# Schatten2021/rust-raytracing

Hardware: AMD Instinct MI355X
Metric: Mrays/s (primary rays, whole node), 10k-sphere 1080p 64spp (higher is better)
Workload: dtype f64; 1 GPU; C2: 10k random spheres (scene seed 1), 1920x1080, 64 spp; width=1920, height=1080, rays_per_pixel=64, n_objects=10000, partition=single GPU

## Files before the change

rust-raytracing_amd/build.py:

```python
import hashlib
import os
import shutil
import subprocess
from concurrent.futures import ThreadPoolExecutor

HERE = os.path.dirname(os.path.abspath(__file__))
CSRC = os.path.join(HERE, "csrc")
LIB = os.path.join(HERE, "librtx_hip.so")
LAB_LIB = os.path.join(HERE, "librtx_hip_lab.so")
OBJ_DIR = os.path.join(HERE, "build")
SOURCES = ["rtx_kernels.hip", "rtx_bvh_spheres.hip", "rtx_bvh_mesh.hip", "rtx_wavefront.hip", "rtx_query.hip", "rtx_update.hip", "rtx_pack.hip",
           "rtx_api.hip", "rtx_api_update.hip", "rtx_api_debug.hip"]
HEADERS = ["rtx_math.h", "rtx_scene.h", "rtx_bvh.h", "rtx_device.h", "rtx_traverse.h", "rtx_mesh_step.h", "rtx_wavefront.h",
           "rtx_launch.h", "rtx_refit.h", "rtx_pack.h", "rtx_host.h"]
FLAGS = ["--offload-arch=gfx950", "-O3", "-std=c++17", "-fPIC", "-ffp-contract=off",
         "-fno-fast-math", "-Wall", "-Wno-unused-function"]
LAB_FLAGS = ["-DRTX_LAB"]


def hipcc():
    exe = shutil.which("hipcc") or "/opt/rocm/bin/hipcc"
    if not os.path.exists(exe):
        raise RuntimeError("hipcc not found: librtx_hip.so cannot be built (there is no CPU fallback)")
    return exe


def _input_files():
    files = [os.path.join(CSRC, f) for f in HEADERS]
    files.append(os.path.join(HERE, "..", "include", "rtx_hip.h"))
    return files


def _digest(source, flags):
    h = hashlib.sha256()
    h.update(" ".join(flags).encode())
    for f in [os.path.join(CSRC, source)] + _input_files():
        with open(f, "rb") as fh:
            h.update(fh.read())
    return h.hexdigest()[:20]


def build(force=False, extra_flags=(), verbose=False, lib=None, jobs=None, lab=False):
    if lib is None:
        lib = LAB_LIB if lab else LIB
    flags = FLAGS + (LAB_FLAGS if lab else []) + list(extra_flags)
    os.makedirs(OBJ_DIR, exist_ok=True)
    exe = hipcc()
    objs, todo = [], []
    for s in SOURCES:
        obj = os.path.join(OBJ_DIR, "%s.%s.o" % (s[:-4], _digest(s, flags)))
        objs.append(obj)
        if force or not os.path.exists(obj):
            todo.append((s, obj))

    def compile_one(job):
        s, obj = job
        cmd = [exe] + flags + ["-c", os.path.join(CSRC, s), "-o", obj + ".tmp"]
        if verbose:
            print(" ".join(cmd), flush=True)
        subprocess.check_call(cmd)
        os.replace(obj + ".tmp", obj)

    if todo:
        with ThreadPoolExecutor(max_workers=jobs or min(len(todo), max(1, (os.cpu_count() or 2) - 1))) as ex:
            list(ex.map(compile_one, todo))
    stamp = lib + ".objs"
    want = "\n".join(os.path.basename(o) for o in objs) + "\n"
    have = open(stamp).read() if os.path.exists(stamp) else None
    if todo or not os.path.exists(lib) or have != want:
        if os.path.exists(stamp):
            os.remove(stamp)
        cmd = [exe, "--offload-arch=gfx950", "-shared", "-fPIC", "-Wl,-Bsymbolic"] + objs + ["-o", lib + ".tmp"]
        if verbose:
            print(" ".join(cmd), flush=True)
        subprocess.check_call(cmd)
        os.replace(lib + ".tmp", lib)
        with open(stamp, "w") as fh:
            fh.write(want)
    if not extra_flags:
        keep = set()
        for st in os.listdir(HERE):
            if st.endswith(".so.objs") and os.path.exists(os.path.join(HERE, st[:-5])):
                keep.update(open(os.path.join(HERE, st)).read().split())
        for f in os.listdir(OBJ_DIR):
            if f.endswith(".o") and f not in keep:
                os.remove(os.path.join(OBJ_DIR, f))
    return lib


def build_all(force=False, verbose=False):
    return build(force=force, verbose=verbose), build(force=force, verbose=verbose, lab=True)


if __name__ == "__main__":
    import sys
    for path in build_all(force="--force" in sys.argv, verbose=True):
        print(path)
# ... 1 lines not shown
```

rust-raytracing_amd/csrc/rtx_bvh_spheres.hip:

```cpp
#include "rtx_launch.h"
#include "rtx_traverse.h"

#include <cmath>

namespace rtx {

#ifndef RTX_SPH_WAVES
#define RTX_SPH_WAVES 4
#endif
constexpr int kSphWavesPerSimd = RTX_SPH_WAVES;
constexpr int kSphStack = 30;

struct SphSurvivor {
    double px, py, pz, dx, dy, dz;
    uint32_t ridx;
    uint32_t first_id;
    uint64_t key;
};
static_assert(sizeof(SphSurvivor) == 64, "SphSurvivor must be one 64-byte line");
struct SphQueue {
    SphSurvivor *rec;
    const uint32_t *perm;
    unsigned long long *count;
    unsigned long long capacity;
    uint32_t cut_walkers;
};
constexpr uint32_t kSphQueueChunk = 512;
#ifndef RTX_SPH_CUT
#define RTX_SPH_CUT 24
#endif
#ifndef RTX_SPH_CUT_DONE
#define RTX_SPH_CUT_DONE 32
#endif
#ifndef RTX_SPH_LEAF_LANES
#define RTX_SPH_LEAF_LANES 8
#endif
#ifndef RTX_ROUND_GLOBAL
#define RTX_ROUND_GLOBAL 1
#endif
#ifndef RTX_ROUND_CARRY_KEY
#define RTX_ROUND_CARRY_KEY 1
#endif
#ifndef RTX_ROUND_DRAW
#define RTX_ROUND_DRAW 1
#endif
constexpr bool kRoundGlobal = RTX_ROUND_GLOBAL != 0;
constexpr uint32_t kSphLeafLanes = RTX_SPH_LEAF_LANES;
constexpr uint32_t kSphCutWalkers = RTX_SPH_CUT;
constexpr uint32_t kSphCutDone = RTX_SPH_CUT_DONE;

__device__ __forceinline__ void sph_queue_append(const SphQueue &sq, Counters *__restrict__ ctr, bool go, const RayState &r,
                                                 uint32_t ridx, uint32_t first_id, uint32_t lane,
                                                 unsigned long long &out_next, unsigned long long &out_end)
{
    const unsigned long long m = __ballot(go);
    const uint32_t n = (uint32_t)__popcll(m);
    if (n == 0u) return;
    const unsigned long long rem = out_end - out_next;
    unsigned long long base2 = 0;
    if (rem < (unsigned long long)n) {
        if (lane == 0) base2 = atomicAdd(sq.count, (unsigned long long)kSphQueueChunk);
        base2 = ((unsigned long long)__builtin_amdgcn_readfirstlane((uint32_t)(base2 >> 32)) << 32) |
                __builtin_amdgcn_readfirstlane((uint32_t)base2);
    }
    if (go) {
        const unsigned long long k = bvh_mbcnt(m);
        const unsigned long long slot = k < rem ? out_next + k : base2 + (k - rem);
        if (slot < sq.capacity) {
            double4 *p = reinterpret_cast<double4 *>(sq.rec + slot);
            p[0] = make_double4(r.pos.x, r.pos.y, r.pos.z, r.dir.x);
            uint2 tail;
            tail.x = ridx; tail.y = first_id;
#if RTX_ROUND_CARRY_KEY
            p[1] = make_double4(r.dir.y, r.dir.z, __longlong_as_double(((long long)tail.y << 32) | (long long)tail.x),
                                __longlong_as_double((long long)r.key));
#else
            p[1] = make_double4(r.dir.y, r.dir.z, __longlong_as_double(((long long)tail.y << 32) | (long long)tail.x), 0.0);
#endif
        } else {
            atomicAdd(&ctr[1].pad_, 1ull);
        }
    }
    if (rem < (unsigned long long)n) { out_next = base2 + ((unsigned long long)n - rem); out_end = base2 + kSphQueueChunk; }
// ... 176 lines not shown
            }
            if (RTX_SPH_PROFILE == 8 && alive && !midwalk && walked && !overflow) rtx_prof += qcnt;
        }
#endif
        if (alive && !midwalk) {
            Hit h;
            hit_init(h);
            ++segs;
            box_tests += nbox;
            leaf_filters += nleaf;
            if (walked && !overflow) {
#pragma unroll 1
                for (uint32_t e = 0; e < qcnt; ++e) {
                    if (__uint_as_float(lq[(size_t)(kSphQueue + e) * kBvhThreads + tid]) <= best_up) {
                        const uint32_t idx = lq[(size_t)e * kBvhThreads + tid];
                        double t;
                        if (sphere_distance(la.spheres[idx], rx, &t)) hit_consider(h, t, la.sphere_ids[idx], 0, idx);
                        exact += 1;
                    }
                }
            } else {
                for (uint32_t k = 0; k < sv.n_spheres; ++k) {
                    double t;
                    if (sphere_distance(la.spheres[k], rx, &t)) hit_consider(h, t, la.sphere_ids[k], 0, k);
                }
                exact += sv.n_spheres;
            }
            for (uint32_t k = 0; k < sv.n_planes; ++k) {
                double t;
                if (plane_distance(sv.planes[k], rx, &t)) hit_consider(h, t, sv.planes[k].id, 1, k);
            }
            for (uint32_t k = 0; k < sv.n_tri_filter; ++k) {
                const uint32_t tk = la.tri_fidx[k];
                double t;
                if (triangle_distance(la.tris[tk], rx, &t)) hit_consider(h, t, la.tris[tk].id, 2, tk);
            }
            exact += sv.n_planes + sv.n_tri_filter;

            bool done = true;
            if (h.id != kNone) {
#if RTX_ROUND_DRAW
                r.draw = 6u + 2u * r.bounce;
#endif
                advance_and_shade<kRoundGlobal>(sv, h, r);
                first_id = h.id;
                done = (r.bounce >= bounce_limit) || light_is_zero(r);
            }
            if (done) {
                store_sample<kRoundGlobal>(samples, rv, ridx, r.result);
                alive = false;
            }
        }
        if constexpr (MODE == 1) {
            sph_queue_append(sq, ctr, alive, r, ridx, first_id, lane, out_next, out_end);
            alive = false;
        }
    }
    if constexpr (MODE == 1) sph_queue_close(sq, lane, out_next, out_end);
#if defined(RTX_LAB) && defined(RTX_SPH_PROFILE)
    if (MODE == 2) exact = rtx_prof;
#endif
    unsigned long long filt = box_tests + leaf_filters;
#pragma unroll
    for (int off = 32; off > 0; off >>= 1) {
        segs += __shfl_xor(segs, off, 64);
        exact += __shfl_xor(exact, off, 64);
        filt += __shfl_xor(filt, off, 64);
        box_tests += __shfl_xor(box_tests, off, 64);
    }
    if (lane == 0) {
        const uint32_t shard = (blockIdx.x * (kBvhThreads >> 6) + (tid >> 6)) & (kCounterShards - 1);
        if (segs) atomicAdd(&ctr[shard].segments, segs);
        if (exact) atomicAdd(&ctr[shard].exact_tests, exact);
        if (filt) atomicAdd(&ctr[shard].filter_tests, filt);
        if (box_tests) atomicAdd(&ctr[2 + (shard % (kCounterShards - 2))].pad_, box_tests);
    }
}

constexpr int kSpkStack = 63;
#ifndef RTX_SPK_WAVES
#define RTX_SPK_WAVES 4
#endif
constexpr int kSpkWaves = RTX_SPK_WAVES;
#ifdef RTX_LAB
constexpr uint32_t kSphNoPackets = 1u;
#endif



template <int SGN>
__device__ __forceinline__ void sph_packet_walk(const PkConst4 cnodes, const PkConst4 csph, const PkConstU32 cprims, uint32_t root,
                                                const Ray32S &q, const SphereRay &sr, uint32_t *lq, uint32_t tid, uint32_t lane,
                                                float &best_up, uint32_t &qcnt, bool &overflow, uint32_t &nbox, uint32_t &nleaf)
{
    int stk = 0;
    uint32_t sp = 0, node = __builtin_amdgcn_readfirstlane(root);
    while (node != kNone) {
        const PkConst4 np = cnodes + 8 * (size_t)node;
        float4 a[4], b[4];
#pragma unroll
        for (int c = 0; c < 4; ++c) { a[c] = np[c]; b[c] = np[4 + c]; }
        uint32_t lnk[4], cnt[4];
        float tc[4];
        unsigned long long hm[4];
#pragma unroll
        for (int c = 0; c < 4; ++c) {
            lnk[c] = pk_bits(a[c].w);
            cnt[c] = pk_bits(b[c].w);
            float tn, tf;
            if (SGN < 8) {
                const float nx_ = (SGN & 1) ? b[c].x : a[c].x, fx_ = (SGN & 1) ? a[c].x : b[c].x;
                const float ny_ = (SGN & 2) ? b[c].y : a[c].y, fy_ = (SGN & 2) ? a[c].y : b[c].y;
                const float nz_ = (SGN & 4) ? b[c].z : a[c].z, fz_ = (SGN & 4) ? a[c].z : b[c].z;
                tn = fmaxf(fmaxf(__builtin_fmaf(nx_, q.ix, q.nx), __builtin_fmaf(ny_, q.iy, q.ny)), fmaxf(__builtin_fmaf(nz_, q.iz, q.nz), 0.0f));
                tf = fminf(fminf(__builtin_fmaf(fx_, q.ix, q.nx), __builtin_fmaf(fy_, q.iy, q.ny)), __builtin_fmaf(fz_, q.iz, q.nz));
            } else {
                const float x0 = __builtin_fmaf(a[c].x, q.ix, q.nx), x1 = __builtin_fmaf(b[c].x, q.ix, q.nx);
                const float y0 = __builtin_fmaf(a[c].y, q.iy, q.ny), y1 = __builtin_fmaf(b[c].y, q.iy, q.ny);
                const float z0 = __builtin_fmaf(a[c].z, q.iz, q.nz), z1 = __builtin_fmaf(b[c].z, q.iz, q.nz);
                tn = fmaxf(fmaxf(fminf(x0, x1), fminf(y0, y1)), fmaxf(fminf(z0, z1), 0.0f));
                tf = fminf(fminf(fmaxf(x0, x1), fmaxf(y0, y1)), fmaxf(z0, z1));
            }
            tc[c] = __builtin_fmaf(tn, 1.0f - 4.76837158e-7f, -q.e);
            const float tf_hi = __builtin_fmaf(tf, 1.0f + 4.76837158e-7f, q.e);
            hm[c] = __builtin_amdgcn_ballot_w64(tc[c] <= fminf(tf_hi, best_up));
        }
        if (best_up >= 0.0f) nbox += 4;
        if (((cnt[0] | cnt[1] | cnt[2] | cnt[3]) & 0xFFFFu) != 0u) {
            uint32_t leafmask = 0;
#pragma unroll
            for (int c = 0; c < 4; ++c)
                if (cnt[c] - 1u < 0xFFFFu && hm[c] != 0ull) leafmask |= 1u << c;
            while (leafmask != 0u) {
                const uint32_t c = (uint32_t)__builtin_ctz(leafmask);
                leafmask &= leafmask - 1u;
                const uint32_t first = c == 0 ? lnk[0] : (c == 1 ? lnk[1] : (c == 2 ? lnk[2] : lnk[3]));
                const uint32_t n = (c == 0 ? cnt[0] : (c == 1 ? cnt[1] : (c == 2 ? cnt[2] : cnt[3]))) & 0xFFFFu;
                const unsigned long long m = c == 0 ? hm[0] : (c == 1 ? hm[1] : (c == 2 ? hm[2] : hm[3]));
                const bool in = ((m >> lane) & 1ull) != 0ull;
                if (in) nleaf += n;
                for (uint32_t j = 0; j < n; ++j) {
                    const float4 rec = csph[first + j];
                    const uint32_t prim = cprims[first + j];
                    if (!in) continue;
                    sph_packet_leaf_test(rec, prim, sr, lq, tid, best_up, qcnt, overflow);
                }
            }
#pragma unroll
            for (int c = 0; c < 4; ++c) hm[c] &= __builtin_amdgcn_ballot_w64(tc[c] <= best_up);
        }
#ifndef RTX_SPK_FAST1
#define RTX_SPK_FAST1 2
#endif
#if RTX_SPK_FAST1
        {
            uint32_t ib = 0;
#pragma unroll
            for (int c = 0; c < 4; ++c) ib |= (cnt[c] == 0u && hm[c] != 0ull) ? 1u << c : 0u;
            if ((ib & (ib - 1u)) == 0u) {
                node = ib == 0u ? kNone : (ib == 1u ? lnk[0] : (ib == 2u ? lnk[1] : (ib == 4u ? lnk[2] : lnk[3])));
                if (node == kNone && sp != 0u) {
                    sp -= 1;
                    node = (uint32_t)__builtin_amdgcn_readlane(stk, (int)sp);
                }
                continue;
            }
#if RTX_SPK_FAST1 >= 2
            if (__builtin_popcount(ib) == 2) {
                uint32_t far_link = 0;
#define RTX_SPK_PAIR(A, B)                                                                                                        \
                {                                                                                                                   \
                    const int ka = (int)__builtin_amdgcn_readlane(__float_as_uint(tc[A]), (int)__builtin_ctzll(hm[A]));            \
                    const int kb = (int)__builtin_amdgcn_readlane(__float_as_uint(tc[B]), (int)__builtin_ctzll(hm[B]));            \
                    const bool sw = kb < ka;                                                                                        \
                    node = sw ? lnk[B] : lnk[A];                                                                                    \
                    far_link = sw ? lnk[A] : lnk[B];                                                                                \
                }
                switch (ib) {
                    case 3u: RTX_SPK_PAIR(0, 1) break;
                    case 5u: RTX_SPK_PAIR(0, 2) break;
                    case 9u: RTX_SPK_PAIR(0, 3) break;
                    case 6u: RTX_SPK_PAIR(1, 2) break;
                    case 10u: RTX_SPK_PAIR(1, 3) break;
                    default: RTX_SPK_PAIR(2, 3) break;
                }
#undef RTX_SPK_PAIR
                stk = rtx_writelane((int)far_link, (int)sp, stk);
                sp += 1u;
                continue;
            }
#endif
        }
#endif
        int key[4];
        uint32_t kl[4];
        constexpr int kFar = 0x7F800000;
#pragma unroll
        for (int c = 0; c < 4; ++c) {
            const unsigned long long m = cnt[c] == 0u ? hm[c] : 0ull;
            const int k = (int)__builtin_amdgcn_readlane(__float_as_uint(tc[c]), (int)__builtin_ctzll(m | 0x8000000000000000ull));
            key[c] = m != 0ull ? k : kFar;
            kl[c] = lnk[c];
        }
#define RTX_CSWAP(i, j) { if (key[j] < key[i]) { int tk = key[i]; key[i] = key[j]; key[j] = tk; uint32_t tl = kl[i]; kl[i] = kl[j]; kl[j] = tl; } }
        RTX_CSWAP(0, 1) RTX_CSWAP(2, 3) RTX_CSWAP(0, 2) RTX_CSWAP(1, 3) RTX_CSWAP(1, 2)
#undef RTX_CSWAP
        stk = rtx_writelane((int)kl[3], (int)sp, stk); sp += key[3] < kFar ? 1u : 0u;
        stk = rtx_writelane((int)kl[2], (int)sp, stk); sp += key[2] < kFar ? 1u : 0u;
        stk = rtx_writelane((int)kl[1], (int)sp, stk); sp += key[1] < kFar ? 1u : 0u;
        node = key[0] < kFar ? kl[0] : kNone;
        if (node == kNone && sp != 0u) {
            sp -= 1;
            node = (uint32_t)__builtin_amdgcn_readlane(stk, (int)sp);
        }
    }
}


__global__ __launch_bounds__(kBvhThreads, kSpkWaves) void trace_sph_packet_kernel(const SceneView *__restrict__ svp,
                                                                                  const RowsView *__restrict__ rvp,
                                                                                  double *__restrict__ samples, Counters *__restrict__ ctr,
                                                                                  unsigned long long *__restrict__ work_counter,
                                                                                  const float4 *__restrict__ nodes, const LeafArrays la,
                                                                                  const SphQueue sq, const TileLists tl)
{
    const SceneView &sv = *svp;
    const RowsView &rv = *rvp;
    __shared__ uint32_t lds_q[2 * kSphQueue][kBvhThreads];
    uint32_t *const lq = &lds_q[0][0];
    const uint32_t tid = threadIdx.x, lane = tid & 63u;
    const uint32_t bounce_limit = sv.max_bounces >= 0xFFFFFFF0ull ? 0xFFFFFFF0u : (uint32_t)sv.max_bounces + 1u;
    const unsigned long long n_rays = rv.n_rays;
    const PkConst4 cnodes = pk_const(nodes), csph = pk_const(la.sphere_f32);
    const PkConstU32 cprims = pk_const(la.sphere_prims);
    unsigned long long wave_next = 0, wave_end = 0;
    unsigned long long out_next = 0, out_end = 0;
    unsigned long long segs = 0, box_tests = 0, leaf_filters = 0, exact = 0;

#ifndef RTX_SPK_GRAB_MUL
#define RTX_SPK_GRAB_MUL 2
#endif
    const unsigned long long pk_grab = (unsigned long long)rv.grab * RTX_SPK_GRAB_MUL;
    for (;;) {
        if (wave_next >= wave_end) {
            unsigned long long base = 0;
            if (lane == 0) base = atomicAdd(work_counter, pk_grab);
            base = ((unsigned long long)__builtin_amdgcn_readfirstlane((uint32_t)(base >> 32)) << 32) |
                   __builtin_amdgcn_readfirstlane((uint32_t)base);
            if (base >= n_rays) break;
            wave_next = base;
            wave_end = base + pk_grab < n_rays ? base + pk_grab : n_rays;
        }
        const unsigned long long my = wave_next + lane;
        wave_next += 64ull;
        uint32_t pl = 0, smp = 0;
        bool alive = ray_index_to_pixel_tiled(rv, my, pl, smp);
        RayState r;
        if (alive) gen_primary(sv, rv, pl, rv.sample_begin + smp, r);
        else { r.pos = mk(0., 0., 0.); r.dir = mk(1., 0., 0.); r.result = mk(0., 0., 0.); r.light = mk(1., 1., 1.); r.key = 0; r.draw = 6; r.bounce = 0; }
        const uint32_t ridx = (uint32_t)my;
        const RayX rx = make_rayx(r.pos, r.dir);

        float best_up = -__builtin_inff();
        uint32_t qcnt = 0, nbox = 0, nleaf = 0;
        bool overflow = false, walked = false;
        Ray32S q;
        SphereRay sr;
        q.ix = q.iy = q.iz = 1.0f; q.nx = q.ny = q.nz = 0.0f; q.e = 0.0f;
        sr.px = sr.py = sr.pz = sr.dx = sr.dy = sr.dz = sr.Kg = sr.K = 0.f; sr.c0 = __builtin_inff();
        if (alive) {
            const float omax = fmaxf(fmaxf(__builtin_fabsf((float)r.pos.x), __builtin_fabsf((float)r.pos.y)),
                                     __builtin_fabsf((float)r.pos.z));
            const bool in32 = omax <= sv.bvh_origin_limit;
            if (in32 || omax <= sv.bvh_origin_limit * kBvhRange64) {
                sphere_ray_from(sv, r.pos, r.dir, sr);
                Ray32 q0;
                make_ray32(r.pos, rx.dirn, (double)sv.bvh_inv_max, q0);
                q.ix = q0.ix; q.iy = q0.iy; q.iz = q0.iz; q.nx = q0.nx; q.ny = q0.ny; q.nz = q0.nz;
                q.e = ray32_slack(q0, in32);
                best_up = __builtin_inff();
                walked = true;
            }
        }
        const unsigned long long wm = __ballot(walked);
        uint32_t list_n = kTileListWalk;
        const uint32_t tile_of = __builtin_amdgcn_readfirstlane((uint32_t)(((uint32_t)my - smp * rv.div_per_sample.d) >> 6));
        if (tl.count != nullptr && wm != 0ull) list_n = pk_const(tl.count)[tile_of];
        if (wm != 0ull && list_n != kTileListWalk) {
            const PkConst4 ent = pk_const(reinterpret_cast<const float4 *>(tl.entries + (size_t)tile_of * kTileListCap));
            for (uint32_t k = 0; k < list_n; ++k) {
                const float4 rec = ent[2 * k], tail = ent[2 * k + 1];
                const float t_lb = tail.y;
                const bool in = walked && t_lb <= best_up;
                if (__ballot(in) == 0ull) break;
                if (in) {
                    nleaf += 1;
                    sph_packet_leaf_test(rec, __float_as_uint(tail.x), sr, lq, tid, best_up, qcnt, overflow);
                }
            }
        } else if (wm != 0ull) {
            const uint32_t my_sgn = (q.ix < 0.0f ? 1u : 0u) | (q.iy < 0.0f ? 2u : 0u) | (q.iz < 0.0f ? 4u : 0u);
            const uint32_t sgn = __builtin_amdgcn_readlane(my_sgn, (int)(__ffsll((long long)wm) - 1));
            const uint32_t oct = __ballot(walked && my_sgn != sgn) == 0ull ? sgn : 8u;
#define RTX_SPK_WALK(S) sph_packet_walk<S>(cnodes, csph, cprims, sv.bvh_root, q, sr, lq, tid, lane, best_up, qcnt, overflow, nbox, nleaf)
            switch (oct) {
                case 0: RTX_SPK_WALK(0); break;
                case 1: RTX_SPK_WALK(1); break;
                case 2: RTX_SPK_WALK(2); break;
                case 3: RTX_SPK_WALK(3); break;
                case 4: RTX_SPK_WALK(4); break;
                case 5: RTX_SPK_WALK(5); break;
                case 6: RTX_SPK_WALK(6); break;
                case 7: RTX_SPK_WALK(7); break;
                default: RTX_SPK_WALK(8); break;
            }
#undef RTX_SPK_WALK
        }
        uint32_t first_id = 0;
        if (alive) {
            Hit h;
            hit_init(h);
            ++segs;
            box_tests += nbox;
            leaf_filters += nleaf;
            if (walked && !overflow) {
#pragma unroll 1
                for (uint32_t e = 0; e < qcnt; ++e) {
                    if (__uint_as_float(lq[(size_t)(kSphQueue + e) * kBvhThreads + tid]) <= best_up) {
                        const uint32_t idx = lq[(size_t)e * kBvhThreads + tid];
                        double t;
                        if (sphere_distance(la.spheres[idx], rx, &t)) hit_consider(h, t, la.sphere_ids[idx], 0, idx);
                        exact += 1;
                    }
                }
            } else {
                for (uint32_t k = 0; k < sv.n_spheres; ++k) {
                    double t;
                    if (sphere_distance(la.spheres[k], rx, &t)) hit_consider(h, t, la.sphere_ids[k], 0, k);
                }
                exact += sv.n_spheres;
            }
            for (uint32_t k = 0; k < sv.n_planes; ++k) {
                double t;
                if (plane_distance(sv.planes[k], rx, &t)) hit_consider(h, t, sv.planes[k].id, 1, k);
            }
            for (uint32_t k = 0; k < sv.n_tri_filter; ++k) {
                const uint32_t tk = la.tri_fidx[k];
                double t;
                if (triangle_distance(la.tris[tk], rx, &t)) hit_consider(h, t, la.tris[tk].id, 2, tk);
            }
            exact += sv.n_planes + sv.n_tri_filter;

            bool done = true;
            if (h.id != kNone) {
                advance_and_shade<kRoundGlobal>(sv, h, r);
                first_id = h.id;
                done = (r.bounce >= bounce_limit) || light_is_zero(r);
            }
            if (done) {
                store_sample<kRoundGlobal>(samples, rv, ridx, r.result);
                alive = false;
            }
        }
        sph_queue_append(sq, ctr, alive, r, ridx, first_id, lane, out_next, out_end);
    }
    sph_queue_close(sq, lane, out_next, out_end);
    unsigned long long filt = box_tests + leaf_filters;
#pragma unroll
    for (int off = 32; off > 0; off >>= 1) {
        segs += __shfl_xor(segs, off, 64);
        exact += __shfl_xor(exact, off, 64);
        filt += __shfl_xor(filt, off, 64);
        box_tests += __shfl_xor(box_tests, off, 64);
    }
    if (lane == 0) {
        const uint32_t shard = (blockIdx.x * (kBvhThreads >> 6) + (tid >> 6)) & (kCounterShards - 1);
        if (segs) atomicAdd(&ctr[shard].segments, segs);
        if (exact) atomicAdd(&ctr[shard].exact_tests, exact);
        if (filt) atomicAdd(&ctr[shard].filter_tests, filt);
        if (box_tests) atomicAdd(&ctr[2 + (shard % (kCounterShards - 2))].pad_, box_tests);
    }
}

uint32_t bvh_spheres_spill_entries(const SceneView &sv)
{
    const uint32_t need = 3u * sv.bvh_depth + 2u;
    return need > (uint32_t)kSphStack ? need - (uint32_t)kSphStack : 0u;
}

size_t bvh_spheres_spill_bytes(const SceneView &sv, int n_cus)
{
    return (size_t)bvh_spheres_spill_entries(sv) * (size_t)n_cus * kSphWavesPerSimd * kBvhThreads * sizeof(uint32_t);
}

static uint64_t sph_queue_capacity(uint64_t n_rays, int n_cus)
{
    const int wpc = kSphWavesPerSimd > kSpkWaves ? kSphWavesPerSimd : kSpkWaves;
    return n_rays + (uint64_t)n_cus * wpc * (kBvhThreads / 64) * kSphQueueChunk + kSphQueueChunk;
}

size_t bvh_spheres_tile_list_bytes(uint64_t rays_per_sample)
{
    const uint64_t n_tiles = rays_per_sample >> 6;
    return (size_t)(((n_tiles * sizeof(uint32_t) + 255) & ~(uint64_t)255) + n_tiles * kTileListCap * sizeof(TileEntry));
}

size_t bvh_spheres_queue_bytes(uint64_t n_rays, int n_cus)
{
    const uint64_t cap = sph_queue_capacity(n_rays, n_cus);
    return (size_t)(cap * sizeof(SphSurvivor) + 2 * 256);
}

static bool sph_packets_ok(const SceneView &sv, bool tiled)
{
    return tiled && 3u * sv.bvh_depth + 2u <= (uint32_t)kSpkStack;
}

bool bvh_spheres_two_stage_ok(const SceneView &sv, bool tiled)
{
#ifdef RTX_LAB
    (void)sv; (void)tiled;
    return true;
#else
    return sph_packets_ok(sv, tiled);
#endif
}

hipError_t launch_trace_bvh_spheres(const SceneView *d_sv, const SceneView &sv, const RowsView *d_rv, const RowsView &rv,
                                    double *samples, Counters *counters, unsigned long long *work_counter, uint32_t *spill, int n_cus,
                                    void *queue_mem, uint32_t flags, hipStream_t stream, Counters *stage1_snapshot, hipEvent_t stage1_done,
                                    void *tile_list_mem, bool build_tile_lists)
{
    const uint64_t want = (rv.n_rays + kBvhThreads - 1) / kBvhThreads;
    const uint64_t cap = (uint64_t)n_cus * kSphWavesPerSimd;
    const uint32_t blocks = (uint32_t)(want < cap ? want : cap);
    if (blocks == 0) return hipSuccess;
    LeafArrays la;
    la.sphere_f32 = sv.bvh_leaf_cr; la.sphere_prims = sv.bvh_prims; la.spheres = sv.spheres; la.sphere_ids = sv.sphere_id;
    la.tri_f32 = sv.tri_f32; la.tri_fidx = sv.tri_fidx; la.tris = sv.tris;
    const uint32_t spill_entries = spill ? bvh_spheres_spill_entries(sv) : 0u;
    const bool deep = spill_entries != 0u;
    const float4 *nodes = reinterpret_cast<const float4 *>(sv.bvh_nodes);
    SphQueue sq{};
    sq.cut_walkers = (sv.tuning & RTX_TUNE_NO_CUT) != 0u ? 0u : kSphCutWalkers;
    const float4 *q3nodes = reinterpret_cast<const float4 *>(sv.bvh_q3nodes);
#ifdef RTX_LAB
    const bool q3 = (sv.bvh_flags & 16u) != 0u && sv.bvh_q3nodes != nullptr && (sv.tuning & RTX_TUNE_NO_QNODES) == 0u;
// ... 69 lines not shown
```

rust-raytracing_amd/csrc/rtx_device.h:

```cpp
#pragma once

#include "rtx_bvh.h"
#include "rtx_scene.h"

namespace rtx {

struct SceneView {
    uint64_t rays_per_pixel;
    uint64_t max_bounces;
    double   focal_length, focal_offset, non_focal_offset;
    uint64_t seed;
    V3 cam_pos;
    V3 to_world_x, to_world_y, to_world_z;
    uint32_t n_objects, n_spheres, n_planes, n_tris;
    const SphereX  *spheres;
    const uint32_t *sphere_id;
    const PlaneX   *planes;
    const TriX     *tris;
    const MaterialX *materials;
    const float4   *tri_f32;
    const uint32_t *tri_fidx;
    const float4   *tri_geo;
    uint32_t        n_tri_filter;
    uint32_t        pad0_;
// ... 116 lines not shown
    return *p;
}

template <bool GLOBAL>
__device__ __forceinline__ void atomic_or_u32(uint32_t *p, uint32_t v)
{
#if defined(__HIP_DEVICE_COMPILE__)
    if constexpr (GLOBAL) {
        (void)__hip_atomic_fetch_or((uint32_t __attribute__((address_space(1))) *)p, v, __ATOMIC_RELAXED, __HIP_MEMORY_SCOPE_AGENT);
        return;
    }
#endif
    atomicOr(p, v);
}

__device__ __forceinline__ void ray_index_to_pixel(const RowsView &rv, uint64_t i, uint32_t &pl, uint32_t &s_local)
{
    s_local = fastdiv((uint32_t)i, rv.div_npix);
    pl = (uint32_t)i - s_local * rv.npix;
}

__device__ __forceinline__ bool ray_index_to_pixel_tiled(const RowsView &rv, uint64_t i, uint32_t &pl, uint32_t &s_local)
{
    s_local = fastdiv((uint32_t)i, rv.div_per_sample);
    const uint32_t r = (uint32_t)i - s_local * rv.div_per_sample.d;
    const uint32_t t = r >> 6, j = r & 63u;
    const uint32_t ty = fastdiv(t, rv.div_tiles_x), tx = t - ty * rv.tiles_x;
    const uint32_t x = tx * 8u + (j & 7u), k = ty * 8u + (j >> 3);
    pl = k * rv.width + x;
    return x < rv.width && k < rv.n_rows;
}

template <bool GLOBAL = false>
__device__ __forceinline__ void store_sample(double *__restrict__ samples, const RowsView &rv, uint64_t ridx, V3 c)
{
    if (c.x == 0.0 && c.y == 0.0 && c.z == 0.0) return;
    double4 *rec = reinterpret_cast<double4 *>(samples) + ridx;
    *rec = make_double4(c.x, c.y, c.z, 0.0);
    const uint64_t bit = rv.nonzero_base + ridx;
    atomic_or_u32<GLOBAL>(rv.nonzero + (bit >> 5), 1u << (uint32_t)(bit & 31u));
}

__device__ __forceinline__ V3 primary_focal_point(const SceneView &sv, const RowsView &rv, uint32_t pl)
{
    const uint32_t k = fastdiv(pl, rv.div_width);
    const uint32_t x = pl - k * rv.width;
    const V3 cam_space_dir = mk(rv.sin_x[x], rv.sin_y[k], rv.cos_x[x] * rv.cos_y[k]);
    const V3 ray_dir = mk(dot(cam_space_dir, sv.to_world_x), dot(cam_space_dir, sv.to_world_y),
                          dot(cam_space_dir, sv.to_world_z));
    return vadd(sv.cam_pos, vmuls(ray_dir, sv.focal_length));
}

__device__ __forceinline__ float round_down_f32_dev(double x)
{
    float f = (float)x;
    if ((double)f > x) f = __uint_as_float(f > 0.0f ? __float_as_uint(f) - 1u : (f < 0.0f ? __float_as_uint(f) + 1u : 0x80000001u));
    return f;
}

__device__ __forceinline__ void gen_primary(const SceneView &sv, const RowsView &rv, uint32_t pl, uint32_t sample,
                                            RayState &r)
{
    uint32_t k = fastdiv(pl, rv.div_width);
    uint32_t x = pl - k * rv.width;
    uint32_t y = image_row(rv, k);
    uint64_t pix = (uint64_t)y * rv.width + x;
    r.key = rng_key(sv.seed, pix, sample);
    V3 rnd1;
    rnd1.x = rng_u01(r.key, 0); rnd1.y = rng_u01(r.key, 1); rnd1.z = rng_u01(r.key, 2);
    V3 ray_position = vadd(sv.cam_pos, vmuls(rnd1, sv.non_focal_offset));
    V3 focal_point = primary_focal_point(sv, rv, pl);
    V3 rnd2;
    rnd2.x = rng_u01(r.key, 3); rnd2.y = rng_u01(r.key, 4); rnd2.z = rng_u01(r.key, 5);
    V3 target_point = vadd(focal_point, vmuls(rnd2, sv.focal_offset));
    V3 ray_direction = vsub(target_point, ray_position);
    r.pos = ray_position;
    r.dir = vnorm(ray_direction);
    r.result = mk(0.0, 0.0, 0.0);
    r.light = mk(1.0, 1.0, 1.0);
    r.draw = 6;
    r.bounce = 0;
}

__device__ __forceinline__ V3 random_direction(double u_z, double u_theta)
{
    double z = u_z * 2.0 - 1.0;
    double theta = u_theta * 2.0 * 3.14159265358979323846;
    double r = sqrt(1.0 - z * z);
    double sn, cs;
    sincos_2pi(theta, &sn, &cs);
    return vnorm(mk(r * cs, r * sn, z));
}

__device__ __forceinline__ V3 random_bounce_dir(V3 ray_dir, V3 surface_normal, double surface_roughness,
                                                double u_z, double u_theta)
{
    V3 random_dir = random_direction(u_z, u_theta);
    V3 reflection_dir = vsub(ray_dir, vmuls(vmuls(surface_normal, 2.0), dot(ray_dir, surface_normal)));
    V3 random_to_reflection_dir = vsub(reflection_dir, random_dir);
    double reflection_mult = 1.0 - surface_roughness;
    V3 final_direction = vadd(random_dir, vmuls(random_to_reflection_dir, reflection_mult));
    final_direction = vnorm(final_direction);
    if (dot(final_direction, surface_normal) > 0.0) return final_direction;
    return vneg(final_direction);
}

template <bool GLOBAL = false>
__device__ __forceinline__ V3 normal_at(const SceneView &sv, const Hit &h, V3 world_pos)
{
    if (h.kind == 0) return sphere_normal_at(load_record<GLOBAL>(sv.spheres + h.local), world_pos);
    if (h.kind == 1) return load_record<GLOBAL>(&sv.planes[h.local].nhat);
    return load_record<GLOBAL>(&sv.tris[h.local].nn);
}

template <bool GLOBAL = false>
__device__ __forceinline__ void advance_and_shade(const SceneView &sv, const Hit &h, RayState &r)
{
    r.pos = vadd(r.pos, vmuls(r.dir, h.t));
    const MaterialX m = load_record<GLOBAL>(sv.materials + h.id);
    double u_z = rng_u01(r.key, r.draw);
    double u_theta = rng_u01(r.key, r.draw + 1);
    r.draw += 2;
    r.dir = random_bounce_dir(r.dir, normal_at<GLOBAL>(sv, h, r.pos), m.roughness, u_z, u_theta);
    r.result = vadd(r.result, vmulv(r.light, m.emission_color));
    r.light = vmulv(r.light, m.base_color);
    r.bounce += 1;
}

__device__ __forceinline__ bool light_is_zero(const RayState &r)
{
    return r.light.x == 0.0 && r.light.y == 0.0 && r.light.z == 0.0;
}

struct FilterParams { float dx, dy, dz, npd, p2x, p2y, p2z, nppE; };

__device__ __forceinline__ void filter_idle(FilterParams &f)
{
    f.dx = f.dy = f.dz = f.npd = f.p2x = f.p2y = f.p2z = 0.0f;
    f.nppE = -3.0e30f;
}

__device__ __forceinline__ void filter_pass_all(FilterParams &f)
{
    f.dx = f.dy = f.dz = f.npd = f.p2x = f.p2y = f.p2z = 0.0f;
    f.nppE = 1.0e30f;
}

__device__ __forceinline__ void filter_from_ray(const SceneView &sv, V3 pos, V3 dir, FilterParams &f)
{
    double px = pos.x - sv.sphere_center[0];
    double py = pos.y - sv.sphere_center[1];
    double pz = pos.z - sv.sphere_center[2];
    double pp = px * px + py * py + pz * pz;
    double pd = px * dir.x + py * dir.y + pz * dir.z;
    double M = sv.sphere_cmax + sqrt(pp);
    if (!(M < 1.0e14) || !(M > 1.0e-12)) { filter_pass_all(f); return; }
    double E = M * M * (64.0 / 16777216.0);
    f.dx = (float)dir.x; f.dy = (float)dir.y; f.dz = (float)dir.z;
    f.npd = (float)(-pd);
    f.p2x = (float)(2.0 * px); f.p2y = (float)(2.0 * py); f.p2z = (float)(2.0 * pz);
    f.nppE = (float)(E - pp);
}

struct TriFilterParams { float dx, dy, dz, npx, npy, npz, A, pad; };

__device__ __forceinline__ void tri_filter_idle(TriFilterParams &f)
// ... 44 lines not shown
```

rust-raytracing_amd/csrc/rtx_math.h:

```cpp
#pragma once

#include <hip/hip_runtime.h>
#include <stdint.h>
#include <math.h>

#define RTX_HD __host__ __device__ __forceinline__

namespace rtx {

struct V3 { double x, y, z; };

RTX_HD V3 mk(double x, double y, double z) { V3 r; r.x = x; r.y = y; r.z = z; return r; }
RTX_HD V3 vadd(V3 a, V3 b) { return mk(a.x + b.x, a.y + b.y, a.z + b.z); }
RTX_HD V3 vsub(V3 a, V3 b) { return mk(a.x - b.x, a.y - b.y, a.z - b.z); }
RTX_HD V3 vmuls(V3 a, double s) { return mk(a.x * s, a.y * s, a.z * s); }
RTX_HD V3 vmulv(V3 a, V3 b) { return mk(a.x * b.x, a.y * b.y, a.z * b.z); }
RTX_HD V3 vdivs(V3 a, double s) { return mk(a.x / s, a.y / s, a.z / s); }
RTX_HD V3 vneg(V3 a) { return mk(-a.x, -a.y, -a.z); }

RTX_HD double dot(V3 a, V3 b)
{
    double xx = a.x * b.x;
    double yy = a.y * b.y;
    double zz = a.z * b.z;
    double s = xx + yy;
    return s + zz;
}

RTX_HD V3 cross(V3 a, V3 b)
{
    return mk(a.y * b.z - a.z * b.y,
              a.z * b.x - a.x * b.z,
              a.x * b.y - a.y * b.x);
}

RTX_HD double vlen(V3 a)
{
    double xx = a.x * a.x;
    double yy = a.y * a.y;
    double zz = a.z * a.z;
    double s = xx + yy;
    s = s + zz;
    return sqrt(s);
}

RTX_HD V3 vnorm(V3 a) { return vdivs(a, vlen(a)); }

RTX_HD uint64_t mix64(uint64_t z)
{
    z ^= z >> 30; z *= 0xBF58476D1CE4E5B9ULL;
    z ^= z >> 27; z *= 0x94D049BB133111EBULL;
    z ^= z >> 31;
    return z;
}

RTX_HD uint64_t rng_key(uint64_t seed, uint64_t pixel_index, uint64_t sample_index)
{
    uint64_t a = mix64(seed + 0x9E3779B97F4A7C15ULL * (pixel_index + 1));
    return mix64(a ^ (0xD1B54A32D192ED03ULL * (sample_index + 1)));
}

RTX_HD double rng_u01(uint64_t key, uint32_t draw_index)
{
    uint64_t z = mix64(key + 0x9E3779B97F4A7C15ULL * ((uint64_t)draw_index + 1));
    uint64_t bits = 0x3FF0000000000000ULL | (z >> 12);
#if defined(__HIP_DEVICE_COMPILE__)
    return __longlong_as_double((long long)bits) - 1.0;
#else
    double d;
    __builtin_memcpy(&d, &bits, sizeof d);
    return d - 1.0;
#endif
}

RTX_HD void sincos_2pi(double x, double *sn, double *cs)
{
    const double invpio2 = 6.36619772367581382433e-01, pio2_1 = 1.57079632673412561417e+00,
                 pio2_2 = 6.07710050630396597660e-11, pio2_2t = 2.02226624879595063154e-21;
    const double S1 = -1.66666666666666324348e-01, S2 = 8.33333333332248946124e-03, S3 = -1.98412698298579493134e-04,
                 S4 = 2.75573137070700676789e-06, S5 = -2.50507602534068634195e-08, S6 = 1.58969099521155010221e-10;
    const double C1 = 4.16666666666666019037e-02, C2 = -1.38888888888741095749e-03, C3 = 2.48015872894767294178e-05,
                 C4 = -2.75573143513906633035e-07, C5 = 2.08757232129817482790e-09, C6 = -1.13596475577881948265e-11;
    const double fn = rint(x * invpio2);
    const double r1 = x - fn * pio2_1, w2 = fn * pio2_2;
    const double r = r1 - w2;
    const double w = fn * pio2_2t - ((r1 - r) - w2);
    const double y0 = r - w, y1 = (r - y0) - w;
    const double z = y0 * y0, zl = fma(y0, y0, -z);
    const double v = z * y0, vl = fma(z, y0, -v) + zl * y0;
    const double rs = S2 + z * (S3 + z * (S4 + z * (S5 + z * S6)));
    double sm = z * (v * rs - 0.5 * y1) + y1;
    sm = fma(vl, S1, sm);
    sm = fma(v, S1, sm);
    const double s = y0 + sm;
    const double rc = z * (C1 + z * (C2 + z * (C3 + z * (C4 + z * (C5 + z * C6)))));
    const double h = 0.5 * z, w1 = 1.0 - h;
    double cm = fma(z, rc, -(y0 * y1));
    cm = fma(-0.5, zl, cm);
    cm = ((1.0 - w1) - h) + cm;
    const double c = w1 + cm;
    const int n = (int)fn & 3;
    *sn = n == 0 ? s : (n == 1 ? c : (n == 2 ? -s : -c));
    *cs = n == 0 ? c : (n == 1 ? -s : (n == 2 ? -c : s));
}

RTX_HD bool is_normal_positive(double d)
{
    return d >= 2.2250738585072014e-308 && d <= 1.7976931348623157e308;
}

}
```

Baseline: 4151 Mrays/s.

## Schedule sphere packet work as tile-sample units and hoist per-pixel ray setup

Replaces linear ray-range grabbing in the sphere packet kernel with work units made of one 64-ray tile and a run of consecutive samples. The per-pixel decode, RNG pixel hash, focal point and tile-list count are computed once per unit and reused across its samples. Construction of the 32-bit traversal ray is also deferred so it only happens when the BVH walk path runs, not the tile-list path. The cost is a new unit-decoding scheme with a different work order and atomic granularity, which may change load balance and cache locality across tiles.

```diff
diff --git a/rust-raytracing_amd/build.py b/rust-raytracing_amd/build.py
--- a/rust-raytracing_amd/build.py
+++ b/rust-raytracing_amd/build.py
@@ -12,7 +12,7 @@
 SOURCES = ["rtx_kernels.hip", "rtx_bvh_spheres.hip", "rtx_bvh_mesh.hip", "rtx_wavefront.hip", "rtx_query.hip", "rtx_update.hip", "rtx_pack.hip",
            "rtx_api.hip", "rtx_api_update.hip", "rtx_api_debug.hip"]
 HEADERS = ["rtx_math.h", "rtx_scene.h", "rtx_bvh.h", "rtx_device.h", "rtx_traverse.h", "rtx_mesh_step.h", "rtx_wavefront.h",
-           "rtx_launch.h", "rtx_refit.h", "rtx_pack.h", "rtx_host.h"]
+           "rtx_launch.h", "rtx_refit.h", "rtx_pack.h", "rtx_host.h", "rtx_spk_units.h"]
 FLAGS = ["--offload-arch=gfx950", "-O3", "-std=c++17", "-fPIC", "-ffp-contract=off",
          "-fno-fast-math", "-Wall", "-Wno-unused-function"]
 LAB_FLAGS = ["-DRTX_LAB"]
diff --git a/rust-raytracing_amd/csrc/rtx_bvh_spheres.hip b/rust-raytracing_amd/csrc/rtx_bvh_spheres.hip
--- a/rust-raytracing_amd/csrc/rtx_bvh_spheres.hip
+++ b/rust-raytracing_amd/csrc/rtx_bvh_spheres.hip
@@ -1,4 +1,5 @@
 #include "rtx_launch.h"
+#include "rtx_spk_units.h"
 #include "rtx_traverse.h"
 
 #include <cmath>
@@ -341,6 +342,12 @@
 #define RTX_SPK_WAVES 4
 #endif
 constexpr int kSpkWaves = RTX_SPK_WAVES;
+#ifndef RTX_SPK_LAZY_RAY
+#define RTX_SPK_LAZY_RAY 1
+#endif
+#ifndef RTX_SPK_UNITS
+#define RTX_SPK_UNITS 1
+#endif
 #ifdef RTX_LAB
 constexpr uint32_t kSphNoPackets = 1u;
 #endif
@@ -492,7 +499,9 @@
     const unsigned long long n_rays = rv.n_rays;
     const PkConst4 cnodes = pk_const(nodes), csph = pk_const(la.sphere_f32);
     const PkConstU32 cprims = pk_const(la.sphere_prims);
+#if !RTX_SPK_UNITS
     unsigned long long wave_next = 0, wave_end = 0;
+#endif
     unsigned long long out_next = 0, out_end = 0;
     unsigned long long segs = 0, box_tests = 0, leaf_filters = 0, exact = 0;
 
@@ -500,8 +509,43 @@
 #define RTX_SPK_GRAB_MUL 2
 #endif
     const unsigned long long pk_grab = (unsigned long long)rv.grab * RTX_SPK_GRAB_MUL;
+#if RTX_SPK_UNITS
+    const uint32_t per_sample = rv.div_per_sample.d, n_tiles = per_sample >> 6;
+    const uint32_t unit_run = (uint32_t)(pk_grab >> 6) != 0u ? (uint32_t)(pk_grab >> 6) : 1u;
+    const unsigned long long n_units = n_rays != 0ull ? spk_unit_count(n_tiles, rv.n_samples, unit_run) : 0ull;
+#endif
     for (;;) {
-        if (wave_next >= wave_end) {
+#if RTX_SPK_UNITS
+        unsigned long long unit = 0;
+        if (lane == 0) unit = atomicAdd(work_counter, 1ull);
+        unit = ((unsigned long long)__builtin_amdgcn_readfirstlane((uint32_t)(unit >> 32)) << 32) |
+               __builtin_amdgcn_readfirstlane((uint32_t)unit);
+        if (unit >= n_units) break;
+        const SpkUnit wu = spk_unit((uint32_t)unit, n_tiles, rv.n_samples, unit_run);
+        const uint32_t tile_of = wu.tile;
+        uint32_t list_n = kTileListWalk;
+        if (tl.count != nullptr) list_n = pk_const(tl.count)[tile_of];
+        const uint32_t tile_ray = tile_of * 64u + lane;
+        uint32_t pl = 0, smp0 = 0;
+        const bool valid = ray_index_to_pixel_tiled(rv, tile_ray, pl, smp0);
+        uint64_t pixel_half = 0;
+        V3 focal_point = mk(0., 0., 0.);
+        if (valid) {
+            const uint32_t k = fastdiv(pl, rv.div_width), x = pl - k * rv.width;
+            pixel_half = rng_key_pixel(sv.seed, (uint64_t)image_row(rv, k) * rv.width + x);
+            focal_point = primary_focal_point(sv, rv, pl);
+        }
+        const PkConst4 ent = pk_const(reinterpret_cast<const float4 *>(tl.entries + (size_t)tile_of * kTileListCap));
+#pragma unroll 1
+        for (uint32_t us = 0; us < wu.count; ++us) {
+            const uint32_t smp = wu.first + us;
+            const uint32_t ridx = smp * per_sample + tile_ray;
+            bool alive = valid;
+            RayState r;
+            if (alive) gen_primary_at(sv, pixel_half, focal_point, rv.sample_begin + smp, r);
+            else { r.pos = mk(0., 0., 0.); r.dir = mk(1., 0., 0.); r.result = mk(0., 0., 0.); r.light = mk(1., 1., 1.); r.key = 0; r.draw = 6; r.bounce = 0; }
+#else
+        {
             unsigned long long base = 0;
             if (lane == 0) base = atomicAdd(work_counter, pk_grab);
             base = ((unsigned long long)__builtin_amdgcn_readfirstlane((uint32_t)(base >> 32)) << 32) |
@@ -510,118 +554,134 @@
             wave_next = base;
             wave_end = base + pk_grab < n_rays ? base + pk_grab : n_rays;
         }
-        const unsigned long long my = wave_next + lane;
-        wave_next += 64ull;
-        uint32_t pl = 0, smp = 0;
-        bool alive = ray_index_to_pixel_tiled(rv, my, pl, smp);
-        RayState r;
-        if (alive) gen_primary(sv, rv, pl, rv.sample_begin + smp, r);
-        else { r.pos = mk(0., 0., 0.); r.dir = mk(1., 0., 0.); r.result = mk(0., 0., 0.); r.light = mk(1., 1., 1.); r.key = 0; r.draw = 6; r.bounce = 0; }
-        const uint32_t ridx = (uint32_t)my;
-        const RayX rx = make_rayx(r.pos, r.dir);
-
-        float best_up = -__builtin_inff();
-        uint32_t qcnt = 0, nbox = 0, nleaf = 0;
-        bool overflow = false, walked = false;
-        Ray32S q;
-        SphereRay sr;
-        q.ix = q.iy = q.iz = 1.0f; q.nx = q.ny = q.nz = 0.0f; q.e = 0.0f;
-        sr.px = sr.py = sr.pz = sr.dx = sr.dy = sr.dz = sr.Kg = sr.K = 0.f; sr.c0 = __builtin_inff();
-        if (alive) {
-            const float omax = fmaxf(fmaxf(__builtin_fabsf((float)r.pos.x), __builtin_fabsf((float)r.pos.y)),
-                                     __builtin_fabsf((float)r.pos.z));
-            const bool in32 = omax <= sv.bvh_origin_limit;
-            if (in32 || omax <= sv.bvh_origin_limit * kBvhRange64) {
-                sphere_ray_from(sv, r.pos, r.dir, sr);
-                Ray32 q0;
-                make_ray32(r.pos, rx.dirn, (double)sv.bvh_inv_max, q0);
-                q.ix = q0.ix; q.iy = q0.iy; q.iz = q0.iz; q.nx = q0.nx; q.ny = q0.ny; q.nz = q0.nz;
-                q.e = ray32_slack(q0, in32);
-                best_up = __builtin_inff();
-                walked = true;
-            }
-        }
-        const unsigned long long wm = __ballot(walked);
-        uint32_t list_n = kTileListWalk;
-        const uint32_t tile_of = __builtin_amdgcn_readfirstlane((uint32_t)(((uint32_t)my - smp * rv.div_per_sample.d) >> 6));
-        if (tl.count != nullptr && wm != 0ull) list_n = pk_const(tl.count)[tile_of];
-        if (wm != 0ull && list_n != kTileListWalk) {
+        for (; wave_next < wave_end; wave_next += 64ull) {
+            const unsigned long long my = wave_next + lane;
+            uint32_t pl = 0, smp = 0;
+            bool alive = ray_index_to_pixel_tiled(rv, my, pl, smp);
+            uint32_t list_n = kTileListWalk;
+            const uint32_t tile_of = __builtin_amdgcn_readfirstlane((uint32_t)(((uint32_t)my - smp * rv.div_per_sample.d) >> 6));
+            if (tl.count != nullptr) list_n = pk_const(tl.count)[tile_of];
             const PkConst4 ent = pk_const(reinterpret_cast<const float4 *>(tl.entries + (size_t)tile_of * kTileListCap));
-            for (uint32_t k = 0; k < list_n; ++k) {
-                const float4 rec = ent[2 * k], tail = ent[2 * k + 1];
-                const float t_lb = tail.y;
-                const bool in = walked && t_lb <= best_up;
-                if (__ballot(in) == 0ull) break;
-                if (in) {
-                    nleaf += 1;
-                    sph_packet_leaf_test(rec, __float_as_uint(tail.x), sr, lq, tid, best_up, qcnt, overflow);
-                }
-            }
-        } else if (wm != 0ull) {
-            const uint32_t my_sgn = (q.ix < 0.0f ? 1u : 0u) | (q.iy < 0.0f ? 2u : 0u) | (q.iz < 0.0f ? 4u : 0u);
-            const uint32_t sgn = __builtin_amdgcn_readlane(my_sgn, (int)(__ffsll((long long)wm) - 1));
-            const uint32_t oct = __ballot(walked && my_sgn != sgn) == 0ull ? sgn : 8u;
+            RayState r;
+            if (alive) gen_primary(sv, rv, pl, rv.sample_begin + smp, r);
+            else { r.pos = mk(0., 0., 0.); r.dir = mk(1., 0., 0.); r.result = mk(0., 0., 0.); r.light = mk(1., 1., 1.); r.key = 0; r.draw = 6; r.bounce = 0; }
+            const uint32_t ridx = (uint32_t)my;
+#endif
+            const RayX rx = make_rayx(r.pos, r.dir);
+
+            float best_up = -__builtin_inff();
+            uint32_t qcnt = 0, nbox = 0, nleaf = 0;
+            bool overflow = false, walked = false, in32 = false;
+            SphereRay sr;
+            sr.px = sr.py = sr.pz = sr.dx = sr.dy = sr.dz = sr.Kg = sr.K = 0.f; sr.c0 = __builtin_inff();
+#if !RTX_SPK_LAZY_RAY
+            Ray32S q;
+            q.ix = q.iy = q.iz = 1.0f; q.nx = q.ny = q.nz = 0.0f; q.e = 0.0f;
+#endif
+            if (alive) {
+                const float omax = fmaxf(fmaxf(__builtin_fabsf((float)r.pos.x), __builtin_fabsf((float)r.pos.y)),
+                                         __builtin_fabsf((float)r.pos.z));
+                in32 = omax <= sv.bvh_origin_limit;
+                if (in32 || omax <= sv.bvh_origin_limit * kBvhRange64) {
+                    sphere_ray_from(sv, r.pos, r.dir, sr);
+#if !RTX_SPK_LAZY_RAY
+                    Ray32 q0;
+                    make_ray32(r.pos, rx.dirn, (double)sv.bvh_inv_max, q0);
+                    q.ix = q0.ix; q.iy = q0.iy; q.iz = q0.iz; q.nx = q0.nx; q.ny = q0.ny; q.nz = q0.nz;
+                    q.e = ray32_slack(q0, in32);
+#endif
+                    best_up = __builtin_inff();
+                    walked = true;
+                }
+            }
+            const unsigned long long wm = __ballot(walked);
+            if (wm != 0ull && list_n != kTileListWalk) {
+                for (uint32_t k = 0; k < list_n; ++k) {
+                    const float4 rec = ent[2 * k], tail = ent[2 * k + 1];
+                    const float t_lb = tail.y;
+                    const bool in = walked && t_lb <= best_up;
+                    if (__ballot(in) == 0ull) break;
+                    if (in) {
+                        nleaf += 1;
+                        sph_packet_leaf_test(rec, __float_as_uint(tail.x), sr, lq, tid, best_up, qcnt, overflow);
+                    }
+                }
+            } else if (wm != 0ull) {
+#if RTX_SPK_LAZY_RAY
+                Ray32S q;
+                q.ix = q.iy = q.iz = 1.0f; q.nx = q.ny = q.nz = 0.0f; q.e = 0.0f;
+                if (walked) {
+                    Ray32 q0;
+                    make_ray32(r.pos, rx.dirn, (double)sv.bvh_inv_max, q0);
+                    q.ix = q0.ix; q.iy = q0.iy; q.iz = q0.iz; q.nx = q0.nx; q.ny = q0.ny; q.nz = q0.nz;
+                    q.e = ray32_slack(q0, in32);
+                }
+#endif
+                const uint32_t my_sgn = (q.ix < 0.0f ? 1u : 0u) | (q.iy < 0.0f ? 2u : 0u) | (q.iz < 0.0f ? 4u : 0u);
+                const uint32_t sgn = __builtin_amdgcn_readlane(my_sgn, (int)(__ffsll((long long)wm) - 1));
+                const uint32_t oct = __ballot(walked && my_sgn != sgn) == 0ull ? sgn : 8u;
 #define RTX_SPK_WALK(S) sph_packet_walk<S>(cnodes, csph, cprims, sv.bvh_root, q, sr, lq, tid, lane, best_up, qcnt, overflow, nbox, nleaf)
-            switch (oct) {
-                case 0: RTX_SPK_WALK(0); break;
-                case 1: RTX_SPK_WALK(1); break;
-                case 2: RTX_SPK_WALK(2); break;
-                case 3: RTX_SPK_WALK(3); break;
-                case 4: RTX_SPK_WALK(4); break;
-                case 5: RTX_SPK_WALK(5); break;
-                case 6: RTX_SPK_WALK(6); break;
-                case 7: RTX_SPK_WALK(7); break;
-                default: RTX_SPK_WALK(8); break;
-            }
+                switch (oct) {
+                    case 0: RTX_SPK_WALK(0); break;
+                    case 1: RTX_SPK_WALK(1); break;
+                    case 2: RTX_SPK_WALK(2); break;
+                    case 3: RTX_SPK_WALK(3); break;
+                    case 4: RTX_SPK_WALK(4); break;
+                    case 5: RTX_SPK_WALK(5); break;
+                    case 6: RTX_SPK_WALK(6); break;
+                    case 7: RTX_SPK_WALK(7); break;
+                    default: RTX_SPK_WALK(8); break;
+                }
 #undef RTX_SPK_WALK
-        }
-        uint32_t first_id = 0;
-        if (alive) {
-            Hit h;
-            hit_init(h);
-            ++segs;
-            box_tests += nbox;
-            leaf_filters += nleaf;
-            if (walked && !overflow) {
+            }
+            uint32_t first_id = 0;
+            if (alive) {
+                Hit h;
+                hit_init(h);
+                ++segs;
+                box_tests += nbox;
+                leaf_filters += nleaf;
+                if (walked && !overflow) {
 #pragma unroll 1
-                for (uint32_t e = 0; e < qcnt; ++e) {
-                    if (__uint_as_float(lq[(size_t)(kSphQueue + e) * kBvhThreads + tid]) <= best_up) {
-                        const uint32_t idx = lq[(size_t)e * kBvhThreads + tid];
+                    for (uint32_t e = 0; e < qcnt; ++e) {
+                        if (__uint_as_float(lq[(size_t)(kSphQueue + e) * kBvhThreads + tid]) <= best_up) {
+                            const uint32_t idx = lq[(size_t)e * kBvhThreads + tid];
+                            double t;
+                            if (sphere_distance(la.spheres[idx], rx, &t)) hit_consider(h, t, la.sphere_ids[idx], 0, idx);
+                            exact += 1;
+                        }
+                    }
+                } else {
+                    for (uint32_t k = 0; k < sv.n_spheres; ++k) {
                         double t;
-                        if (sphere_distance(la.spheres[idx], rx, &t)) hit_consider(h, t, la.sphere_ids[idx], 0, idx);
-                        exact += 1;
+                        if (sphere_distance(la.spheres[k], rx, &t)) hit_consider(h, t, la.sphere_ids[k], 0, k);
                     }
-                }
-            } else {
-                for (uint32_t k = 0; k < sv.n_spheres; ++k) {
+                    exact += sv.n_spheres;
+                }
+                for (uint32_t k = 0; k < sv.n_planes; ++k) {
                     double t;
-                    if (sphere_distance(la.spheres[k], rx, &t)) hit_consider(h, t, la.sphere_ids[k], 0, k);
-                }
-                exact += sv.n_spheres;
-            }
-            for (uint32_t k = 0; k < sv.n_planes; ++k) {
-                double t;
-                if (plane_distance(sv.planes[k], rx, &t)) hit_consider(h, t, sv.planes[k].id, 1, k);
-            }
-            for (uint32_t k = 0; k < sv.n_tri_filter; ++k) {
-                const uint32_t tk = la.tri_fidx[k];
-                double t;
-                if (triangle_distance(la.tris[tk], rx, &t)) hit_consider(h, t, la.tris[tk].id, 2, tk);
-            }
-            exact += sv.n_planes + sv.n_tri_filter;
-
-            bool done = true;
-            if (h.id != kNone) {
-                advance_and_shade<kRoundGlobal>(sv, h, r);
-                first_id = h.id;
-                done = (r.bounce >= bounce_limit) || light_is_zero(r);
-            }
-            if (done) {
-                store_sample<kRoundGlobal>(samples, rv, ridx, r.result);
-                alive = false;
-            }
-        }
-        sph_queue_append(sq, ctr, alive, r, ridx, first_id, lane, out_next, out_end);
+                    if (plane_distance(sv.planes[k], rx, &t)) hit_consider(h, t, sv.planes[k].id, 1, k);
+                }
+                for (uint32_t k = 0; k < sv.n_tri_filter; ++k) {
+                    const uint32_t tk = la.tri_fidx[k];
+                    double t;
+                    if (triangle_distance(la.tris[tk], rx, &t)) hit_consider(h, t, la.tris[tk].id, 2, tk);
+                }
+                exact += sv.n_planes + sv.n_tri_filter;
+
+                bool done = true;
+                if (h.id != kNone) {
+                    advance_and_shade<kRoundGlobal>(sv, h, r);
+                    first_id = h.id;
+                    done = (r.bounce >= bounce_limit) || light_is_zero(r);
+                }
+                if (done) {
+                    store_sample<kRoundGlobal>(samples, rv, ridx, r.result);
+                    alive = false;
+                }
+            }
+            sph_queue_append(sq, ctr, alive, r, ridx, first_id, lane, out_next, out_end);
+        }
     }
     sph_queue_close(sq, lane, out_next, out_end);
     unsigned long long filt = box_tests + leaf_filters;
diff --git a/rust-raytracing_amd/csrc/rtx_device.h b/rust-raytracing_amd/csrc/rtx_device.h
--- a/rust-raytracing_amd/csrc/rtx_device.h
+++ b/rust-raytracing_amd/csrc/rtx_device.h
@@ -222,6 +222,24 @@
     r.bounce = 0;
 }
 
+__device__ __forceinline__ void gen_primary_at(const SceneView &sv, uint64_t pixel_half, V3 focal_point, uint32_t sample, RayState &r)
+{
+    r.key = rng_key_sample(pixel_half, sample);
+    V3 rnd1;
+    rnd1.x = rng_u01(r.key, 0); rnd1.y = rng_u01(r.key, 1); rnd1.z = rng_u01(r.key, 2);
+    V3 ray_position = vadd(sv.cam_pos, vmuls(rnd1, sv.non_focal_offset));
+    V3 rnd2;
+    rnd2.x = rng_u01(r.key, 3); rnd2.y = rng_u01(r.key, 4); rnd2.z = rng_u01(r.key, 5);
+    V3 target_point = vadd(focal_point, vmuls(rnd2, sv.focal_offset));
+    V3 ray_direction = vsub(target_point, ray_position);
+    r.pos = ray_position;
+    r.dir = vnorm(ray_direction);
+    r.result = mk(0.0, 0.0, 0.0);
+    r.light = mk(1.0, 1.0, 1.0);
+    r.draw = 6;
+    r.bounce = 0;
+}
+
 __device__ __forceinline__ V3 random_direction(double u_z, double u_theta)
 {
     double z = u_z * 2.0 - 1.0;
diff --git a/rust-raytracing_amd/csrc/rtx_math.h b/rust-raytracing_amd/csrc/rtx_math.h
--- a/rust-raytracing_amd/csrc/rtx_math.h
+++ b/rust-raytracing_amd/csrc/rtx_math.h
@@ -60,6 +60,9 @@
     return mix64(a ^ (0xD1B54A32D192ED03ULL * (sample_index + 1)));
 }
 
+RTX_HD uint64_t rng_key_pixel(uint64_t seed, uint64_t pixel_index) { return mix64(seed + 0x9E3779B97F4A7C15ULL * (pixel_index + 1)); }
+RTX_HD uint64_t rng_key_sample(uint64_t pixel_half, uint64_t sample_index) { return mix64(pixel_half ^ (0xD1B54A32D192ED03ULL * (sample_index + 1))); }
+
 RTX_HD double rng_u01(uint64_t key, uint32_t draw_index)
 {
     uint64_t z = mix64(key + 0x9E3779B97F4A7C15ULL * ((uint64_t)draw_index + 1));
diff --git a/rust-raytracing_amd/csrc/rtx_spk_units.h b/rust-raytracing_amd/csrc/rtx_spk_units.h
--- /dev/null
+++ b/rust-raytracing_amd/csrc/rtx_spk_units.h
@@ -0,0 +1,32 @@
+#pragma once
+
+#include <stdint.h>
+
+#if defined(__HIPCC__) || defined(__CUDACC__)
+#define RTX_SPK_HD __host__ __device__ inline
+#else
+#define RTX_SPK_HD inline
+#endif
+
+namespace rtx {
+
+struct SpkUnit { uint32_t tile, first, count; };
+
+RTX_SPK_HD uint32_t spk_runs_per_tile(uint32_t n_samples, uint32_t group) { return (n_samples + group - 1u) / group; }
+
+RTX_SPK_HD uint64_t spk_unit_count(uint32_t n_tiles, uint32_t n_samples, uint32_t group)
+{
+    return (uint64_t)n_tiles * spk_runs_per_tile(n_samples, group);
+}
+
+RTX_SPK_HD SpkUnit spk_unit(uint32_t u, uint32_t n_tiles, uint32_t n_samples, uint32_t group)
+{
+    const uint32_t run = u / n_tiles;
+    SpkUnit w;
+    w.tile = u - run * n_tiles;
+    w.first = run * group;
+    w.count = n_samples - w.first < group ? n_samples - w.first : group;
+    return w;
+}
+
+}
```

Result: faster. 4239 Mrays/s, median of 6 (+2.1%).
